# mayataka/robotoc

Measured on AMD Instinct MI355X. Metric: riccati_sweeps_per_sec, higher is better.
Workload: dtype f64; 1 GPU; anymal_trot_N40 (nv=18,nu=12, 47 grids: 2 lifts + 2 impacts, switching constraints ns=6), 4096 DISTINCT OCP instances per GPU (randomised stage data and dx0), backward+forward Riccati sweep; per_gpu_batch=4096, stages=47, parallelism=instances sharded, dp1

## Files before the change

### robotoc_amd/csrc/kernel_set.hpp

```cpp
#pragma once
#include <cstring>

#include "../../include/rtoc.h"
#include "kernel_table.hpp"
#include "condense.hpp"
#include "unconstr_dynamics.hpp"
#include "friction_cone.hpp"
#include "riccati_backward.hpp"
#include "riccati_backward_rs.hpp"
#include "riccati_backward_rv.hpp"
#include "riccati_backward_rw.hpp"
#include "riccati_backward_rw2.hpp"
#include "condense_rv.hpp"
#include "riccati_scan.hpp"
#include "riccati_forward.hpp"
#include "unconstr_riccati.hpp"
#include "parnmpc_backward_correction.hpp"

namespace rtoc {

template <int NV, int NU, int NS, int NW0, int NW1>
inline KernelSet make_set() {
  KernelSet k;
  memset(&k, 0, sizeof(k));
  k.nv = NV;
  k.nu = NU;
  k.ns = NS;
  k.nvariants = 2;
  k.kl = StaticLayout<NV, NU, NS>::make().kkt;
  k.rl = StaticLayout<NV, NU, NS>::make().ric;
  k.bwd[0] = {riccati_backward_kernel<NV, NU, NS, NW0>, 64 * NW0, BwdCfg<NV, NU, NS, NW0>::LDS_BYTES, 1};
  k.bwd[1] = {riccati_backward_kernel<NV, NU, NS, NW1>, 64 * NW1, BwdCfg<NV, NU, NS, NW1>::LDS_BYTES, 1};
  if constexpr (2 * NV + 1 <= 64 && NU + 3 <= 16 && rs_rider_columns_fit<NV>) {
    k.bwd[2] = {riccati_backward_rs_kernel<NV, NU, NS>, 128, BwdCfg<NV, NU, NS, 2>::LDS_BYTES, 1};
    k.nvariants = 3;
    if (4 * BwdCfg<NV, NU, NS, 2>::LDS_BYTES + 64 <= 160 * 1024) {
      k.bwd[3] = {riccati_backward_rs4_kernel<NV, NU, NS>, 512, 4 * BwdCfg<NV, NU, NS, 2>::LDS_BYTES + 64, 4};
      k.nvariants = 4;
      if constexpr (NV % 4 == 2 && NV > NU) k.bwd_sa = {riccati_backward_rs4_kernel<NV, NU, NS, true>, 512, k.bwd[3].lds, 4};
    }
  }
  if constexpr (RvCfg<NV, NU>::OK) {
    k.bwd_rv = {riccati_backward_rv_kernel<NV, NU, NS, false>, 64, rv_lds_bytes<NV, NU, NS>(), 1};
    if constexpr (NV % 16 == 2 && RvCfg<NV, NU>::T == 3 && NV - NU > 0 && NV - NU <= 8 && (NV - NU) % 2 == 0)
    {
      k.bwd_rv_sa = {riccati_backward_rv_kernel<NV, NU, NS, true>, 64, k.bwd_rv.lds, 1};
      k.bwd_rv_sto = {riccati_backward_rv_kernel<NV, NU, NS, true, true>, 64, k.bwd_rv.lds, 1};
    }
  }
  if constexpr (RwCfg<NV, NU>::OK)
    k.bwd_rw = {riccati_backward_rw_kernel<NV, NU, NS>, 64, RwLds<NV, NU, NS>::BYTES, 1};
  else if constexpr (RwCfg<NV, NU>::OK2)
    k.bwd_rw = {riccati_backward_rw2_kernel<NV, NU, NS>, 128, Rw2Lds<NV, NU, NS>::BYTES, 1};
  constexpr int NWF = (2 * NV + NU + 63) / 64;
  if constexpr (NWF == 1)
    k.fwd = {riccati_forward_kernel<NV, NU, NS>, 64, 0, 1};
  else
    k.fwd = {riccati_forward_mw_kernel<NV, NU, NS, NWF>, 64 * NWF, 0, 1};
  k.dl = StaticLayout<NV, NU, NS>::make().dir;
  k.cl = StaticLayout<NV, NU, NS>::make().cdd;
  k.fill = {unconstr_fill_kernel<NV>, 128, 0, 1};
  k.ucond = {unconstr_condense_kernel<NV>, 64, 0, 1};
  k.uexp = {unconstr_expand_kernel<NV>, 64, 0, 1};
  if constexpr (NU == NV && NS == 0 && 2 * NV + 1 <= 64) {
    if constexpr (NV <= 8) k.ubwd = {unconstr_riccati_backward_kernel<NV>, 64, 0, 1};
    else k.ubwd = {unconstr_riccati_backward_lds_kernel<NV>, 64, 0, 1};
    k.ufwd = {unconstr_riccati_forward_kernel<NV>, 64, 0, 1};
  }
  if constexpr (NU == NV && NS == 0 && PbcCfg<NV>::OK) {
    k.pcoarse = {parnmpc_coarse_kernel<NV>, 64, 0, 1};
    k.pcorrect = {parnmpc_correct_kernel<NV>, PBC_CORRECT_NT, 0, 1};
  }
  k.ccond = {cone_condense_kernel<NV, NS>, 64, 0, 1};
  k.cexp = {cone_expand_kernel<NV, NS>, 64, 0, 1};
  k.wcond = {wrench_condense_kernel<NV, NS>, 64, 0, 1};
  k.wexp = {wrench_expand_kernel<NV, NS>, 64, 0, 1};
  constexpr int NF = NS;
  k.cond = {condense_kernel<NV, NU, NF, NS>, CondCfg<NV, NU, NF, NS>::NT, CondCfg<NV, NU, NF, NS>::LDS_BYTES, 1};
  k.cond_split = {condense_kernel<NV, NU, NF, NS, true>, CondCfg<NV, NU, NF, NS>::NT, CondCfg<NV, NU, NF, NS, true>::LDS_BYTES, 1};
  k.mjt = {mjtjinv_kernel<NV, NU, NF, NS>, 64, MjCfg<NV, NF>::LDS_BYTES, 1};
  k.cond_fuses_cones = CondCfg<NV, NU, NF, NS>::FUSE ? 1 : 0;
  k.cond_fused_default = (CondCfg<NV, NU, NF, NS>::FUSE && CondCfg<NV, NU, NF, NS>::ITEMS >= 5) ? 1 : 0;
  if constexpr (CrvCfg<NV, NU, NF, NS>::OK) {
    k.cond_rv = {condense_rv_kernel<NV, NU, NF, NS>, 64, CrvCfg<NV, NU, NF, NS>::LDS_BYTES, 1};
    k.cond_rv_nc = {condense_rv_kernel<NV, NU, NF, NS, false>, 64, CrvCfg<NV, NU, NF, NS>::LDS_BYTES, 1};
    k.cond_rv_cones = CrvCfg<NV, NU, NF, NS>::CONES ? 1 : 0;
  }
  static_assert(!(NV == 18 && NU == 12 && NS == 12) ||
                    (CondCfg<NV, NU, NF, NS, true>::ITEMS >= 5 && CondCfg<NV, NU, NF, NS, true>::MIN_WAVES == 4 && MjCfg<NV, NF>::ITEMS >= 10),
                "LDS carve of the split condensation grew past its granule budget");
  k.expd = {expand_kernel<NV, NU, NF, NS>, 64, ExpCfg<NV, NU, NF>::LDS_BYTES, 1};
  k.scan_elt = {scan_element_kernel<NV, NU, NS>, SCAN_ELT_NT, scan::ElementCfg<NV, NU, NS>::LDS_BYTES, 1};
  k.scan_comb = {scan_combine_kernel<NV>, scan_comb_nt(NV), scan::CombineCfg<NV, scan_comb_nt(NV)>::LDS_BYTES, 1};
  k.scan_elt_stride = scan::EltLayout<NV>::STRIDE;
  k.scan_ps_stride = scan::EltLayout<NV>::PS_STRIDE;
  k.scan_ps_soff = scan::EltLayout<NV>::PS_S;
  k.scan_policy_variant = 1;
  k.fscan_elt = {fwd_scan_element_kernel<NV, NU, NS>, SCAN_FWD_NT, scan::FwdCfg<NV, NU>::LDS_BYTES, 1};
  k.fscan_comb = {fwd_scan_combine_kernel<NV, NU, NS>, SCAN_FWD_NT, scan::FwdCfg<NV, NU>::LDS_BYTES, 1};
  k.fscan_fin = {fwd_scan_finish_kernel<NV, NU, NS>, 64, 0, 1};
  k.sto_prep = {scan_sto_prep_kernel<NV, NU, NS>, SCAN_STO_PREP_NT, scan::StoPrepCfg<NV, NU, NS>::LDS_DOUBLES * (int)sizeof(double), 1};
  k.sto_vec = {scan_sto_vector_kernel<NV, NU, NS>, scan_sto_vec_nt(NV), scan::StoVecCfg<NV, NU, NS>::LDS_BYTES, 1};
  k.sto_scr_stride = scan::StoScratch<NV, NU, NS>::STRIDE;
  static_assert(scan::StoVecCfg<NV, NU, NS>::LDS_BYTES <= 160 * 1024, "the vector pass keeps one grid point's bundle in LDS");
  static_assert(scan::StoVecCfg<NV, NU, NS>::MAX_STAGES == SCAN_STO_MAX_STAGES, "the host's limit (kernel_args.hpp) is the kernel's grid table");
  static_assert(scan::CombineCfg<NV, scan_comb_nt(NV)>::LDS_BYTES <= 160 * 1024, "combination scratch must fit the LDS of a CU");
  return k;
}


// ... 2 lines not shown
```

### robotoc_amd/csrc/kernel_table.hpp

```cpp
#pragma once
#include <cstddef>

#include "kernel_args.hpp"

namespace rtoc {

template <class Args>
struct Kern {
  void (*fn)(Args);
  int threads;
  int lds;
  int inst;
  constexpr explicit operator bool() const { return fn != nullptr; }
};
constexpr size_t kernel_abi_stamp() {
  size_t h = 1469598103934665603ull;
  const size_t parts[] = {sizeof(BwdArgs), sizeof(FwdArgs), sizeof(FillArgs), sizeof(UdArgs), sizeof(ConeArgs), sizeof(CondArgs),
                          sizeof(ExpArgs), sizeof(ScanArgs), sizeof(FwdScanArgs), sizeof(UrArgs), sizeof(StoScanArgs),
                          sizeof(PbcArgs), sizeof(Kern<BwdArgs>)};
  for (size_t v : parts) h = (h ^ v) * 1099511628211ull;
  return h;
}

struct alignas(8) ShapeInfo {
  int nv, nu, ns;
  int nvariants;
  rtoc_record_layout kl, rl, dl, cl;
  int cond_fuses_cones;
  int cond_fused_default;
  int cond_rv_cones;
  int scan_elt_stride, scan_ps_stride, scan_ps_soff;
  int scan_policy_variant;
  int sto_scr_stride;
};
struct KernelSet : ShapeInfo {
  Kern<BwdArgs> bwd[4];
  Kern<BwdArgs> bwd_sa;
  Kern<BwdArgs> bwd_rv;
  Kern<BwdArgs> bwd_rv_sa;
  Kern<BwdArgs> bwd_rv_sto;
  Kern<BwdArgs> bwd_rw;
  Kern<FwdArgs> fwd;
  Kern<FillArgs> fill;
  Kern<UdArgs> ucond, uexp;
  Kern<UrArgs> ubwd, ufwd;
  Kern<ConeArgs> ccond, cexp;
  Kern<ConeArgs> wcond, wexp;
  Kern<CondArgs> cond;
  Kern<CondArgs> cond_split, mjt;
  Kern<CondArgs> cond_rv;
  Kern<CondArgs> cond_rv_nc;
  Kern<ExpArgs> expd;
  Kern<ScanArgs> scan_elt, scan_comb;
  Kern<FwdScanArgs> fscan_elt, fscan_comb, fscan_fin;
  Kern<StoScanArgs> sto_prep, sto_vec;
  Kern<PbcArgs> pcoarse, pcorrect;
};

template <class Set, class F>
constexpr void for_each_kernel(Set& k, F&& f) {
  for (auto& b : k.bwd) f(b);
  f(k.bwd_sa), f(k.bwd_rv), f(k.bwd_rv_sa), f(k.bwd_rv_sto), f(k.bwd_rw);
  f(k.fwd), f(k.fill), f(k.ucond), f(k.uexp), f(k.ubwd), f(k.ufwd);
  f(k.ccond), f(k.cexp), f(k.wcond), f(k.wexp);
  f(k.cond), f(k.cond_split), f(k.mjt), f(k.cond_rv), f(k.cond_rv_nc), f(k.expd);
  f(k.scan_elt), f(k.scan_comb), f(k.fscan_elt), f(k.fscan_comb), f(k.fscan_fin), f(k.sto_prep), f(k.sto_vec);
  f(k.pcoarse), f(k.pcorrect);
}
constexpr size_t kernels_visited() {
  KernelSet k{};
  size_t n = 0;
  for_each_kernel(k, [&n](const auto&) { ++n; });
  return n;
}
static_assert(sizeof(Kern<BwdArgs>) == sizeof(Kern<StoScanArgs>) && sizeof(KernelSet) == sizeof(ShapeInfo) + kernels_visited() * sizeof(Kern<BwdArgs>),
              "for_each_kernel must visit every descriptor of KernelSet (and KernelSet hold nothing else: plain fields go into ShapeInfo)");

}
```

### robotoc_amd/csrc/riccati_forward.hpp

```cpp
#pragma once
#include "device_utils.hpp"
#include "kernel_args.hpp"
#include "../../include/rtoc.h"

namespace rtoc {

#ifndef FWD_PREFETCH
#define FWD_PREFETCH 12
#endif
#ifndef FWD_WAVES_PER_SIMD
#define FWD_WAVES_PER_SIMD 2
#endif

template <int NV, int NU>
struct FwdPairCfg {
  static constexpr int NX = 2 * NV;
  static constexpr int G = 64 / NV;
  static constexpr int TX = (NX + G - 1) / G;
  static constexpr int TXP = (TX + 1) & ~1;
  static constexpr int TK = (NU + G - 1) / G;
  static constexpr int NVP = (NV + 1) & ~1;
  static constexpr int NF = NV * NU, NFP = (NF + 1) & ~1;
  static constexpr int TF = (NFP + 127) / 128;
};

template <int NWF>
__device__ __forceinline__ void fwd_sync() {
  if constexpr (NWF == 1)
    asm volatile("s_waitcnt lgkmcnt(0)" ::: "memory");
  else
    asm volatile("s_waitcnt lgkmcnt(0)\n\ts_barrier" ::: "memory");
}

template <int NV, int NU, int NS>
__global__ __launch_bounds__(64, FWD_WAVES_PER_SIMD) void riccati_forward_kernel(FwdArgs a) {
  using C = FwdPairCfg<NV, NU>;
  constexpr int NX = C::NX, G = C::G, TX = C::TX, TXP = C::TXP, TK = C::TK, NVP = C::NVP, NF = C::NF, TF = C::TF;
  constexpr int PF = FWD_PREFETCH < TX ? FWD_PREFETCH : TX;
  static_assert(NX + NU <= 64, "one lane per row of [Fxx; K] in the reductions");
  __shared__ __attribute__((aligned(16))) double sDx[2][NX + 8];
  __shared__ __attribute__((aligned(16))) double sXp[2][G * TXP];
  __shared__ __attribute__((aligned(16))) double sPa[G + 1][NX];
  __shared__ __attribute__((aligned(16))) double sPp[G + 1][NX];
  __shared__ __attribute__((aligned(16))) double sPk[NX + NU + 1][NVP];
  __shared__ __attribute__((aligned(16))) double sF[TF * 128];
  __shared__ double sDu[NU + 8];
  __shared__ double sDt[NX];
  __shared__ double sRed[8];
  extern __shared__ int sGridTab[];
  const int tid = threadIdx.x;
  const int b = a.first + blockIdx.x;
  if (b >= a.batch) return;
  for (int st = tid; st < a.nstages; st += 64) {
    const rtoc_grid* gp = a.grid + st;
    sGridTab[st] = (gp->type & 15) | ((gp->sto != 0) << 4) | ((gp->sto_next != 0) << 5) |
                   ((gp->switching_constraint != 0) << 6) | (gp->dims << 8);
  }
  for (int e = tid; e < 2 * G * TXP; e += 64) (&sXp[0][0])[e] = 0.0;
  const int N = a.nstages - 1;
  constexpr rtoc_layout SL = StaticLayout<NV, NU, NS>::make();
  constexpr rtoc_record_layout KL = SL.kkt, RL = SL.ric, DL = SL.dir;
  const double* kb = a.kkt + (size_t)b * a.nstages * KL.stride;
  const double* rb = a.ric + (size_t)b * a.nstages * RL.stride;
  double* db = a.dir + (size_t)b * a.nstages * DL.stride;

  const bool lg = tid < G * NV;
  const int p = lg ? tid % NV : tid - G * NV;
  const int c = lg ? tid / NV : 0;
  const int cw = lg ? c : G;
  const bool xrow = tid < NX;
  const int r = xrow ? tid : NX - 1;
  const bool kl = tid >= NX && tid < NX + NU;
  const int u = kl ? tid - NX : 0;
  const int pos = (r % G) * TXP + r / G;
  __syncthreads();
  if (xrow) {
    const double v = a.dx0 ? a.dx0[(size_t)b * NX + tid] : db[DL.off[RTOC_DIR_DX] + tid];
    sDx[0][tid] = v;
    sXp[0][pos] = v;
    if (a.dx0) db[DL.off[RTOC_DIR_DX] + tid] = v;
  }
  __syncthreads();
  double dts = 0.0, dtsn = 0.0;
  {
    const rtoc_grid g0 = a.grid[0];
    if (g0.sto) {
      if (tid == 0) {
        double acc = 0.0;
        for (int k = 0; k < NX; ++k) acc += rb[RL.off[RTOC_RIC_DTSDX] + k] * sDx[0][k];
        sRed[0] = acc + rb[RL.off[RTOC_RIC_SCAL] + RTOC_RIC_SCAL_DTS0];
      }
      __syncthreads();
      dtsn = sRed[0];
      __syncthreads();
    }
  }
  const int lo = c * NX + 2 * p;
  auto moff = [&](int t) { return (NX % G == 0 || t < TX - 1 || G * t + c < NX) ? lo + t * (G * NX) : (NX - 1) * NX + 2 * p; };
  auto live = [&](int t) { return NX % G == 0 || t < TX - 1 || G * t + c < NX; };
  auto koff = [&](int t) { return (NU % G == 0 || t < TK - 1 || G * t + c < NU) ? lo + t * (G * NX) : (NU - 1) * NX + 2 * p; };
  auto klive = [&](int t) { return NU % G == 0 || t < TK - 1 || G * t + c < NU; };
  const int pe = lg ? c - 2 * p : (1 << 20);
  constexpr unsigned P_SILENT = 0x80000000u;
  const auto prsrc = __builtin_amdgcn_make_buffer_rsrc(const_cast<double*>(rb), 0, a.nstages * (int)RL.stride * 8, 0x00020000);
  const int prow = tid < NX + NU ? tid : NX + NU;
  auto vec_ptr = [&](int st) {
    return xrow ? kb + (size_t)st * KL.stride + KL.off[RTOC_KKT_FX] + tid : rb + (size_t)st * RL.stride + RL.off[RTOC_RIC_KV] + u;
  };
  auto s_ptr = [&](int st) { return rb + (size_t)st * RL.stride + RL.off[RTOC_RIC_S] + r; };
  d2 fa[TX];
  double vec, sv;
#pragma unroll
  for (int t = 0; t < PF; ++t) fa[t] = *(const d2*)(kb + KL.off[RTOC_KKT_FXX] + moff(t));
  vec = *vec_ptr(0);
  sv = *s_ptr(0);
  int cur = 0;
  struct GridBits { int type, sto, sto_next, switching_constraint, dims; };
  for (int st = 0; st < N; ++st) {
    const int gb = __builtin_amdgcn_readfirstlane(sGridTab[st]);
    const GridBits g = {gb & 15, (gb >> 4) & 1, (gb >> 5) & 1, (gb >> 6) & 1, gb >> 8};
    const bool impact = g.type == RTOC_GRID_IMPACT, lift = g.type == RTOC_GRID_LIFT;
    const bool sto = g.sto != 0, sto_next = g.sto_next != 0;
    const double* kr = kb + (size_t)st * KL.stride;
    const double* rr = rb + (size_t)st * RL.stride;
    double* dr = db + (size_t)st * DL.stride;
    const double* dx = sDx[cur];
    const double* xp = sXp[cur];

    if (impact || lift) {
      dts = dtsn;
      dtsn = 0.0;
      if (lift && sto_next) {
        if (tid == 0) {
          double acc = 0.0;
          #pragma unroll 4
          for (int k = 0; k < NX; ++k) acc += rr[RL.off[RTOC_RIC_DTSDX] + k] * dx[k];
          acc += rr[RL.off[RTOC_RIC_SCAL] + RTOC_RIC_SCAL_DTS0];
          if (sto) acc += rr[RL.off[RTOC_RIC_SCAL] + RTOC_RIC_SCAL_DTSDTS] * dts;
          sRed[0] = acc;
        }
        fwd_sync<1>();
        dtsn = sRed[0];
        fwd_sync<1>();
      }
    }

    d2 fk[TK], ff[TF], fp[TX];
#pragma unroll
    for (int t = PF; t < TX; ++t) fa[t] = *(const d2*)(kr + KL.off[RTOC_KKT_FXX] + moff(t));
#pragma unroll
    for (int t = 0; t < TK; ++t) fk[t] = *(const d2*)(rr + RL.off[RTOC_RIC_K] + koff(t));
#pragma unroll
    for (int i = 0; i < TF; ++i) {
      const int e = 2 * (64 * i + tid);
      ff[i] = *(const d2*)(kr + KL.off[RTOC_KKT_FVU] + (e < NF ? e : 0));
    }
    double rd1 = 0.0, rd2 = 0.0, rd3 = 0.0, rdt = 0.0, rs0 = 0.0, rss = 0.0;
    if (sto) {
      rd1 = xrow ? kr[KL.off[RTOC_KKT_FFX] + tid] : rr[RL.off[RTOC_RIC_T] + u];
      rd2 = xrow ? rr[RL.off[RTOC_RIC_PSI] + tid] : rr[RL.off[RTOC_RIC_W] + u];
      rd3 = rr[RL.off[RTOC_RIC_PHI] + r];
    }
    if (impact && sto_next) {
      rdt = rr[RL.off[RTOC_RIC_DTSDX] + r];
      rs0 = rr[RL.off[RTOC_RIC_SCAL] + RTOC_RIC_SCAL_DTS0];
      rss = rr[RL.off[RTOC_RIC_SCAL] + RTOC_RIC_SCAL_DTSDTS];
    }
    d2 x[TXP / 2];
#pragma unroll
    for (int i = 0; i < TXP / 2; ++i) x[i] = *(const d2*)(xp + c * TXP + 2 * i);
    const d2 xq = *(const d2*)(dx + 2 * p);
    double a0 = 0.0, a1 = 0.0;
#pragma unroll
    for (int t = 0; t < TX; ++t) {
      const double xt = x[t / 2][t % 2];
      if (live(t)) {
        a0 += fa[t].x * xt;
        a1 += fa[t].y * xt;
      }
    }
    __builtin_amdgcn_sched_barrier(0);
#pragma unroll
    for (int t = 0; t < TX; ++t) {
      const unsigned vo = (pe + G * t <= 1) ? (unsigned)(lo + t * (G * NX)) * 8u : P_SILENT;
      fp[t] = __builtin_bit_cast(d2, __builtin_amdgcn_raw_buffer_load_b128(prsrc, vo, (unsigned)(st * (int)RL.stride + (int)RL.off[RTOC_RIC_P]) * 8u, 0));
    }
    double pk[TK];
#pragma unroll
    for (int t = 0; t < TK; ++t) pk[t] = fk[t].x * xq.x + fk[t].y * xq.y;
#pragma unroll
    for (int i = 0; i < TF; ++i) *(d2*)(sF + 2 * (64 * i + tid)) = ff[i];
    double q0 = 0.0, q1 = 0.0;
#pragma unroll
    for (int t = 0; t < TX; ++t) {
      const double xt = x[t / 2][t % 2];
      const int dd = pe + G * t;
      const double o0 = q0 + fp[t].x * xt, o1 = q1 + fp[t].y * xt;
      q0 = dd <= 0 ? o0 : q0;
      q1 = dd <= 1 ? o1 : q1;
      const double m1 = fp[t].y * xq.y, m01 = m1 + fp[t].x * xq.x;
      sPk[lg && live(t) ? G * t + c : NX + NU][p] = dd < 0 ? m01 : (dd < 1 ? m1 : 0.0);
    }
    double vec_n, sv_n;
    __builtin_amdgcn_sched_barrier(0);
    {
      const double* kn = kb + (size_t)(st + 1) * KL.stride;
#pragma unroll
      for (int t = 0; t < PF; ++t) fa[t] = *(const d2*)(kn + KL.off[RTOC_KKT_FXX] + moff(t));
      vec_n = *vec_ptr(st + 1);
      sv_n = *s_ptr(st + 1);
    }
    {
      d2 va = {a0, a1}, vp = {q0, q1};
      *(d2*)(&sPa[cw][2 * p]) = va;
      *(d2*)(&sPp[cw][2 * p]) = vp;
#pragma unroll
      for (int t = 0; t < TK; ++t) sPk[lg && klive(t) ? NX + G * t + c : NX + NU][p] = pk[t];
    }
    fwd_sync<1>();
    double acc_a = sPa[0][r], acc_p = sPp[0][r];
#pragma unroll
    for (int cc = 1; cc < G; ++cc) {
      acc_a += sPa[cc][r];
      acc_p += sPp[cc][r];
    }
    double kd = 0.0;
#pragma unroll 3
    for (int i = 0; i < NVP / 2; ++i) {
      const d2 w = *(const d2*)(&sPk[prow][2 * i]);
      kd += w.x;
      if (2 * i + 1 < NV) kd += w.y;
    }
    acc_p += xrow ? kd : 0.0;
    if (kl && !impact) {
      double du = kd + vec;
      if (sto) {
        du += rd1 * (dtsn - dts);
        if (sto_next) du -= rd2 * dtsn;
      }
      sDu[u] = du;
      dr[DL.off[RTOC_DIR_DU] + u] = du;
    }
    fwd_sync<1>();
    double* dxn = sDx[cur ^ 1];
    if (xrow) {
      double v = vec + acc_a;
      if (!impact) {
        if (tid >= NV) {
#pragma unroll 4
          for (int cc = 0; cc < NU; ++cc) v += sF[cc * NV + tid - NV] * sDu[cc];
        }
        if (sto) v += rd1 * (dtsn - dts);
      }
      dxn[tid] = v;
      if (impact && sto_next) sDt[tid] = rdt;
      sXp[cur ^ 1][pos] = v;
      (dr + DL.stride)[DL.off[RTOC_DIR_DX] + tid] = v;
    }
    if (impact && sto_next) {
      fwd_sync<1>();
      if (tid == 0) {
        double acc = 0.0;
        #pragma unroll 4
        for (int k = 0; k < NX; ++k) acc += sDt[k] * dxn[k];
        acc += rs0;
        if (sto) acc += rss * dts;
        sRed[0] = acc;
      }
      fwd_sync<1>();
      dtsn = sRed[0];
    }
    if (xrow) {
      double lam = acc_p - sv;
      if (sto) {
        if (impact) {
          lam -= rd3 * dtsn;
        } else {
          lam += rd2 * (dtsn - dts);
          if (sto_next) lam -= rd3 * dtsn;
        }
      }
      dr[DL.off[RTOC_DIR_DLMDGMM] + tid] = lam;
    }
    if (NS > 0 && g.switching_constraint && tid < g.dims) {
      const double* M = rr + RL.off[RTOC_RIC_M] + tid;
      double acc = 0.0;
      #pragma unroll 4
      for (int j = 0; j < NX; ++j) acc += M[j * NS] * dx[j];
      acc += rr[RL.off[RTOC_RIC_MV] + tid];
      if (sto) {
        acc += rr[RL.off[RTOC_RIC_MT] + tid] * (dtsn - dts);
        if (sto_next) acc -= rr[RL.off[RTOC_RIC_MTN] + tid] * dtsn;
      }
      dr[DL.off[RTOC_DIR_DXI] + tid] = acc;
    }
    if (tid == 0) {
      dr[DL.off[RTOC_DIR_DTS] + 0] = dts;
      dr[DL.off[RTOC_DIR_DTS] + 1] = dtsn;
    }
    fwd_sync<1>();
    cur ^= 1;
    vec = vec_n;
    sv = sv_n;
  }
  {
    const double* rr = rb + (size_t)N * RL.stride;
    double* dr = db + (size_t)N * DL.stride;
    const double* xp = sXp[cur];
    d2 fp[TX], x[TXP / 2];
// ... 213 lines not shown
```

### robotoc_amd/csrc/rt_context.hpp

```cpp
#pragma once
#include <hip/hip_runtime.h>

#include <cstdio>
#include <cstdlib>
#include <cstring>
#include <memory>
#include <new>
#include <string>
#include <vector>

#include "../../include/rtoc.h"
#include "../../include/rtoc_robot.h"
#include "device_buffer.hpp"
#include "kernel_table.hpp"
#include "record_view.hpp"
#include "rigid_body_model.hpp"

#define HIP_TRY(expr)                                 \
  do {                                                \
    hipError_t e_ = (expr);                           \
    if (e_ != hipSuccess) {                           \
      rtoc::ctx_set_err(e_, __FILE_NAME__, __LINE__); \
      return RTOC_ERR_HIP;                            \
    }                                                 \
// ... 41 lines not shown
  CtxStreams() = default;
  CtxStreams(const CtxStreams&) = delete;
  CtxStreams& operator=(const CtxStreams&) = delete;
  ~CtxStreams() {
    if (ev0) (void)hipEventDestroy(ev0);
    if (ev1) (void)hipEventDestroy(ev1);
    if (own_stream) (void)hipStreamDestroy(own_stream);
    if (stream2) (void)hipStreamDestroy(stream2);
    if (ev_fork) (void)hipEventDestroy(ev_fork);
    if (ev_join) (void)hipEventDestroy(ev_join);
    for (hipEvent_t e : ev_chunk)
      if (e) (void)hipEventDestroy(e);
  }
};
struct CtxOptions {
  int writeback = 0;
  double max_dts0 = 0.1;
  double contact_inv_damping = 0.0;
  int bwd_variant = 0;
  int sweep_chunks = 1;
  int condense_split = 0;
  int keep_qaf = 0;
  int fxx_mode = 0;
  int bwd_register = 1;
  int cond_register = 1;
  int use_graph = 0;
  int exact_transport = 0;
  int unconstr_dense = 0;
  int exact_cone_jacobian = 0;
  int impact_cones = 1;
  int linearize_fused = 0;
  int lin_dpp = 0;
  double barrier = 0.0, ftb_rule = 0.0;
  int n_mu = 0;
  bool has_cpos = false, has_crot = false;
  int ls_on = 0;
  double ls_rate = 0.0, ls_min_step = 0.0, ls_cost_rate = 0.0, ls_viol_rate = 0.0;
  int ls_method = 0;
  double ls_armijo = 0.0, ls_margin = 0.0, ls_eps = 0.0;
};
struct GraphSlot {
  hipGraphExec_t exec = nullptr;
  unsigned long long epoch = 0, warm_epoch = 0;
  double p0 = 0.0, p1 = 0.0;
  bool warm = false;
  ~GraphSlot() {
    if (exec) (void)hipGraphExecDestroy(exec);
  }
};


struct SweepState {
  int fxx_state = 0;
  BwdPlan bwd_plan;
  DevBuf<int> d_fxx_flag;
  int backward_scan = 0;
  DevBuf<double> d_scan[3];
  DevBuf<double> d_scan_sto;
};

struct ConstraintState {
  DevBuf<double> d_bounds;
  DevBuf<double> d_mu;
  DevBuf<double> d_wcone;
  void clone_from(const ConstraintState& src, CopyChain& dup) {
    dup(d_bounds, src.d_bounds);
    dup(d_mu, src.d_mu);
    dup(d_wcone, src.d_wcone);
  }
  DevBuf<rtoc_box_row> d_rows;
  std::vector<rtoc_box_row> h_rows;
  DevBuf<int> d_pair;
  DevBuf<int> d_entry;
  int nrows = 0;
  int cone_contacts = 0, cone_dim = 0;
  int cone_rows = 0;
};

struct ModelState {
  DevBuf<rbd::DevModel> d_model;
  std::unique_ptr<rbd::DevModel> h_model;
  DevBuf<unsigned> d_active;
  bool active_current = false;
  DevBuf<double> d_cpos;
  DevBuf<double> d_crot;
  DevBuf<double> d_cost;
  DevBuf<double> d_x0;
  DevBuf<double> d_qtab;
  DevBuf<int> d_qtab_active;
  int qtab_on = 0, qtab_n = 0, qtab_inst = 0;
  bool clone_from(const ModelState& src, CopyChain& dup) {
    if (src.h_model) {
      h_model.reset(new (std::nothrow) rbd::DevModel(*src.h_model));
      if (!h_model) return false;
      dup(d_model, src.d_model);
      if (dup.e == hipSuccess) dup.e = set_linearize_lds(h_model->m, h_model->nlevels, h_model->nbranch, h_model->dpp);
    }
    dup(d_active, src.d_active);
    active_current = src.active_current;
    dup(d_cpos, src.d_cpos);
    dup(d_crot, src.d_crot);
    dup(d_cost, src.d_cost);
    dup(d_x0, src.d_x0);
    qtab_on = src.qtab_on, qtab_n = src.qtab_n, qtab_inst = src.qtab_inst;
    dup(d_qtab, src.d_qtab);
    dup(d_qtab_active, src.d_qtab_active);
    return true;
// ... 240 lines not shown
```

### robotoc_amd/csrc/rt_sweep.hip

```cpp
#include "rt_context.hpp"
#include "fxx_structure.hpp"

using namespace rtoc;

static bool grid_has_sto(const rtoc_ctx* c) {
  for (int i = 0; i < c->nstages; ++i)
    if (c->h_grid[i].sto || c->h_grid[i].sto_next) return true;
  return false;
}
static bool scan_applies(const rtoc_ctx* c) {
  if (!c->backward_scan || c->h_grid.empty()) return false;
  if (c->backward_scan == 2 && c->batch > RTOC_SCAN_AUTO_MAX_BATCH) return false;
  if (c->nstages > SCAN_STO_MAX_STAGES && grid_has_sto(c)) return false;
  return true;
}
static bool forward_scan_applies(const rtoc_ctx* c) { return scan_applies(c) && !grid_has_sto(c); }

int rtoc::ensure_scan_buffers(rtoc_ctx* c) {
  const KernelSet* ks = c->ks;
  const size_t per = (size_t)c->batch * c->max_stages;
  for (int i = 0; i < 3; ++i) HIP_TRY(c->d_scan[i].reserve(per * (i < 2 ? ks->scan_elt_stride : ks->scan_ps_stride)));
  if (grid_has_sto(c)) HIP_TRY(c->d_scan_sto.reserve(per * ks->sto_scr_stride));
  return RTOC_OK;
}
// ... 31 lines not shown
  s.batch = end;
  s.first = first;
  s.dist = 0;
  launch(ks->scan_elt, dim3(n, nb), stream, s);
  int cur = 0;
  for (int d = 1; d < n; d *= 2) {
    s.src = c->d_scan[cur].p;
    s.dst = c->d_scan[cur ^ 1].p;
    s.dist = d;
    launch(ks->scan_comb, dim3(n - d, nb, 2), stream, s);
    cur ^= 1;
  }
  BwdArgs a = bwd_args(c, first, end);
  a.prof = nullptr;
  a.scan_ps = c->d_scan[2].p;
  a.scan_ps_stride = ks->scan_ps_stride;
  a.scan_ps_soff = ks->scan_ps_soff;
  const bool sto = grid_has_sto(c);
  StoScanArgs t;
  const bool ride = sto && !c->writeback && ks->sto_prep.lds <= p.kern->lds;
  if (sto) {
    t.kkt = c->buf[RTOC_BUF_KKT].p, t.ric = c->buf[RTOC_BUF_RIC].p, t.grid = c->d_grid.p, t.status = c->d_status.p;
    t.ps = c->d_scan[2].p, t.scr = c->d_scan_sto.p;
    t.nstages = n, t.batch = end, t.first = first, t.max_dts0 = c->max_dts0, t.prof = c->d_prof.p;
    if (!ride) launch(ks->sto_prep, dim3(n - 1, nb), stream, t);
  }
  a.sto_scr = ride ? c->d_scan_sto.p : nullptr;
  launch(*p.kern, dim3(nb, ride ? 2 * n - 1 : n), stream, a);
  if (sto) launch(ks->sto_vec, dim3(nb), stream, t);
  HIP_TRY(hipGetLastError());
  return RTOC_OK;
}

static int check_fxx(rtoc_ctx* c) {
  HIP_TRY(c->d_fxx_flag.reserve(1));
  HIP_TRY(hipMemsetAsync(c->d_fxx_flag.p, 0, sizeof(int), c->stream));
  FxxCheckArgs a;
  a.kkt = c->buf[RTOC_BUF_KKT].p;
  a.grid = c->d_grid.p;
  a.flag = c->d_fxx_flag.p;
  a.nstages = c->nstages;
  a.batch = c->batch;
  a.nv = c->dims.nv;
  a.np = c->dims.np;
  a.fxx_off = c->L.kkt.off[RTOC_KKT_FXX];
  a.stride = c->L.kkt.stride;
  hipLaunchKernelGGL(fxx_structure_kernel, dim3(c->batch * (c->nstages - 1)), dim3(64), 0, c->stream, a);
  HIP_TRY(hipGetLastError());
  int bad = 1;
  HIP_TRY(hipMemcpyAsync(&bad, c->d_fxx_flag.p, sizeof(int), hipMemcpyDeviceToHost, c->stream));
  HIP_TRY(hipStreamSynchronize(c->stream));
  c->fxx_state = bad ? 2 : 1;
  return RTOC_OK;
}

int rtoc::plan_backward(rtoc_ctx* c, BwdPlan* out) {
  const KernelSet* ks = c->ks;
  const bool reg = c->bwd_register && !c->h_grid.empty() && c->nstages >= 2 && c->nstages <= RV_MAX_STAGES && !c->writeback &&
                   c->bwd_variant == default_bwd_variant(ks);
  const bool sto = reg && grid_has_sto(c);
  const bool rw = reg && ks->bwd_rw && !sto && (c->bwd_register >= 2 || c->batch > c->num_cus);
  const bool rewritable = c->fxx_mode == 0 && (!c->buf[RTOC_BUF_KKT].owned || c->kkt_exposed);
  int rc = RTOC_OK;
  auto structured = [&]() {
    if (!((ks->bwd_sa && c->bwd_variant == 3) || rw) || c->fxx_mode == 1) return false;
    if (c->fxx_mode == 2) return true;
    if (c->fxx_state == 0 && rc == RTOC_OK) rc = check_fxx(c);
    return c->fxx_state == 1;
  };
  BwdPlan p = {BWD_TILE, nullptr, 0};
  if (scan_applies(c)) {
    p = {BWD_SCAN, &ks->bwd[ks->scan_policy_variant], 0};
  } else if (reg && ks->bwd_rv && (!sto || (ks->bwd_rv_sto && structured()))) {
    p.path = BWD_RV;
    p.kern = sto ? &ks->bwd_rv_sto : (ks->bwd_rv_sa && structured()) ? &ks->bwd_rv_sa : &ks->bwd_rv;
    p.check_fxx = (p.kern != &ks->bwd_rv && rewritable) ? 1 : 0;
  } else {
    if (rw && rewritable) c->fxx_state = 0;
    const bool s = structured();
    p.path = (rw && s) ? BWD_RW : BWD_TILE;
    p.kern = (rw && s) ? &ks->bwd_rw : s ? &ks->bwd_sa : &ks->bwd[c->bwd_variant];
  }
  if (rc) return rc;
  if (p.path != c->bwd_plan.path || p.kern != c->bwd_plan.kern || p.check_fxx != c->bwd_plan.check_fxx) c->epoch++;
  c->bwd_plan = *out = p;
  return RTOC_OK;
}

static int launch_backward_rv(rtoc_ctx* c, const BwdPlan& p, int first, int end, hipStream_t stream) {
  const int N = c->nstages - 1;
  BwdArgs a = bwd_args(c, first, end);
  a.seg_hi = N - 1;
  a.seg_lo = 0;
  a.check_fxx = p.check_fxx;
#ifdef RTOC_RV_DEBUG_MASK
  if (const char* e = getenv("RTOC_RV_DEBUG")) a.scan_ps_soff = atoi(e);
#endif
  if (N >= 1) launch(*p.kern, dim3(end - first), stream, a);
  HIP_TRY(hipGetLastError());
  return RTOC_OK;
}

static int launch_backward_rw(rtoc_ctx* c, const BwdPlan& p, int first, int end, hipStream_t stream) {
  const KernelSet* ks = c->ks;
  const int N = c->nstages - 1, nb = end - first;
  BwdArgs a = bwd_args(c, first, end);
  auto constrained = [&](int st) { return c->h_grid[st].type != RTOC_GRID_IMPACT && c->h_grid[st].dims > 0; };
  auto one_stage = [&](int st) {
    BwdArgs o = a;
    o.scan_ps = c->buf[RTOC_BUF_RIC].p + c->L.ric.off[RTOC_RIC_P];
    o.scan_ps_stride = c->L.ric.stride;
    o.scan_ps_soff = c->L.ric.off[RTOC_RIC_S] - c->L.ric.off[RTOC_RIC_P];
    o.seg_hi = o.seg_lo = st;
    launch(ks->bwd[ks->scan_policy_variant], dim3(nb, 1), stream, o);
  };
  if (N == 0 || constrained(N - 1)) one_stage(N);
  int hi = N - 1;
  while (hi >= 0) {
    if (constrained(hi)) {
      one_stage(hi);
      --hi;
      continue;
    }
    int lo = hi;
    while (lo > 0 && !constrained(lo - 1)) --lo;
    a.seg_hi = hi;
    a.seg_lo = lo;
    launch(*p.kern, dim3(nb), stream, a);
    hi = lo - 1;
  }
  HIP_TRY(hipGetLastError());
  return RTOC_OK;
}

static int launch_backward_tile(rtoc_ctx* c, const BwdPlan& p, int first, int end, hipStream_t stream) {
  launch(*p.kern, dim3((end - first + p.kern->inst - 1) / p.kern->inst), stream, bwd_args(c, first, end));
  HIP_TRY(hipGetLastError());
  return RTOC_OK;
// ... 1 lines not shown

static int launch_backward_range(rtoc_ctx* c, const BwdPlan& p, int first, int end, hipStream_t stream) {
  switch (p.path) {
    case BWD_SCAN: return launch_backward_scan(c, p, first, end, stream);
    case BWD_RV: return launch_backward_rv(c, p, first, end, stream);
    case BWD_RW: return launch_backward_rw(c, p, first, end, stream);
    default: return launch_backward_tile(c, p, first, end, stream);
  }
}
int rtoc::launch_backward(rtoc_ctx* c, const BwdPlan& p) { return launch_backward_range(c, p, 0, c->batch, c->stream); }

static int launch_forward_scan(rtoc_ctx* c, int first, int end, hipStream_t stream) {
  const KernelSet* ks = c->ks;
  int rc0 = ensure_scan_buffers(c);
  if (rc0) return rc0;
  const int n = c->nstages, nb = end - first, N = n - 1;
  FwdScanArgs s;
  s.kkt = c->buf[RTOC_BUF_KKT].p;
  s.ric = c->buf[RTOC_BUF_RIC].p;
  s.dir = c->buf[RTOC_BUF_DIR].p;
  s.dx0 = c->buf[RTOC_BUF_DX0].p;
  s.grid = c->d_grid.p;
  s.src = c->d_scan[1].p;
  s.dst = c->d_scan[0].p;
  s.nstages = n;
  s.batch = end;
  s.first = first;
  s.dist = 0;
  launch(ks->fscan_elt, dim3(N, nb), stream, s);
  int cur = 0;
  for (int d = 1; d < N; d *= 2) {
    s.src = c->d_scan[cur].p;
    s.dst = c->d_scan[cur ^ 1].p;
    s.dist = d;
    launch(ks->fscan_comb, dim3(N - d, nb), stream, s);
    cur ^= 1;
  }
  launch(ks->fscan_fin, dim3(n, nb), stream, s);
  HIP_TRY(hipGetLastError());
  return RTOC_OK;
}

static int launch_forward_range(rtoc_ctx* c, int first, int end, hipStream_t stream) {
  if (forward_scan_applies(c)) return launch_forward_scan(c, first, end, stream);
  FwdArgs a;
  a.kkt = c->buf[RTOC_BUF_KKT].p;
  a.ric = c->buf[RTOC_BUF_RIC].p;
  a.dir = c->buf[RTOC_BUF_DIR].p;
  a.dx0 = c->buf[RTOC_BUF_DX0].p;
  a.grid = c->d_grid.p;
  a.nstages = c->nstages;
  a.batch = end;
  a.first = first;
  launch(c->ks->fwd, dim3(end - first), stream, a, ((a.nstages + 3) & ~3) * (int)sizeof(int));
  HIP_TRY(hipGetLastError());
  return RTOC_OK;
}
int rtoc::launch_forward(rtoc_ctx* c) { return launch_forward_range(c, 0, c->batch, c->stream); }

int rtoc::launch_sweep(rtoc_ctx* c, const BwdPlan& p) {
  const int nch = (c->sweep_chunks > 0) ? c->sweep_chunks : 1;
  if (nch == 1 || p.path == BWD_SCAN) {
    int rc = launch_backward(c, p);
    return rc ? rc : launch_forward(c);
  }
  const int per = (((c->batch + nch - 1) / nch) + 3) & ~3;
  HIP_TRY(hipEventRecord(c->ev_fork, c->stream));
  HIP_TRY(hipStreamWaitEvent(c->stream2, c->ev_fork, 0));
  for (int i = 0; i * per < c->batch; ++i) {
    const int first = i * per, end = (first + per < c->batch) ? first + per : c->batch;
    int rc = launch_backward_range(c, p, first, end, c->stream);
    if (rc) return rc;
    hipEvent_t e = c->ev_chunk[i % RTOC_MAX_CHUNK_EVENTS];
    HIP_TRY(hipEventRecord(e, c->stream));
    HIP_TRY(hipStreamWaitEvent(c->stream2, e, 0));
    rc = launch_forward_range(c, first, end, c->stream2);
    if (rc) return rc;
  }
  HIP_TRY(hipEventRecord(c->ev_join, c->stream2));
  HIP_TRY(hipStreamWaitEvent(c->stream, c->ev_join, 0));
  return RTOC_OK;
}

int rtoc_riccati_backward(rtoc_ctx* c) {
  CHECK_READY(c);
  BwdPlan p;
  int rc = plan_backward(c, &p);
  return rc ? rc : launch_backward(c, p);
}

int rtoc_riccati_forward(rtoc_ctx* c) {
  CHECK_READY(c);
  return launch_forward(c);
}

int rtoc_graph_replay_count(rtoc_ctx* c, unsigned long long* out) {
  if (!c || !out) return RTOC_ERR_BAD_ARG;
  *out = c->graph_replays;
  return RTOC_OK;
}

int rtoc_riccati_sweep(rtoc_ctx* c) {
  CHECK_READY(c);
  BwdPlan p;
  int rc = plan_backward(c, &p);
  return rc ? rc : run_graphed(c, &c->g_sweep, 0.0, 0.0, [&]() { return launch_sweep(c, p); });
}
// ... 92 lines not shown
```

### robotoc_amd/csrc/rtoc_capi.hip

```cpp
#include <dlfcn.h>

#include "rt_context.hpp"
#include "device_utils.hpp"

using namespace rtoc;

static thread_local char g_errbuf[256] = "";
void rtoc::ctx_set_err(hipError_t e, const char* file, int line) {
  snprintf(g_errbuf, sizeof(g_errbuf), "HIP error %d (%s) at %s:%d", (int)e, hipGetErrorString(e), file, line);
}

int rtoc_version(void) { return 100; }

int rtoc_device_count(void) {
  int n = 0;
  if (hipGetDeviceCount(&n) != hipSuccess) return 0;
  return n;
}

template <int U, bool COPY>
static __global__ __launch_bounds__(256) void stream_probe_kernel(const char* __restrict__ src, char* __restrict__ dst, size_t chunks,
                                                                  double* sink) {
  const size_t nwaves = (size_t)gridDim.x * 4, w = (size_t)blockIdx.x * 4 + (threadIdx.x >> 6);
  const int lane = threadIdx.x & 63;
// ... 140 lines not shown
}

int rtoc_create(const rtoc_dims* dims, int max_stages, int batch, int device, rtoc_ctx** out) {
  if (!dims || !out || max_stages < 2 || batch < 1) return RTOC_ERR_BAD_ARG;
  const KernelSet* ks = find_set(dims);
  if (!ks) return RTOC_ERR_UNSUPPORTED_DIMS;
  if (rtoc_device_count() <= device || device < 0) return RTOC_ERR_NO_DEVICE;
  HIP_TRY(hipSetDevice(device));
  rtoc_ctx* c = new (std::nothrow) rtoc_ctx();
  if (!c) return RTOC_ERR_BAD_ARG;
  c->device = device;
  int rc = create_members(c, dims, ks, max_stages, batch, device);
  if (rc) {
    (void)rtoc_destroy(c);
    return rc;
  }
  *out = c;
  return RTOC_OK;
}

int rtoc_destroy(rtoc_ctx* c) {
  if (!c) return RTOC_ERR_BAD_ARG;
  (void)hipSetDevice(c->device);
  if (c->stream) (void)hipStreamSynchronize(c->stream);
  delete c;
  return RTOC_OK;
}

int rtoc_clone(rtoc_ctx* c, rtoc_ctx** out) {
  if (!c || !out) return RTOC_ERR_BAD_ARG;
  rtoc_ctx* n = nullptr;
  int rc = rtoc_create(&c->dims, c->max_stages, c->batch, c->device, &n);
  if (rc) return rc;
  if (c->parnmpc) rc = rtoc_parnmpc_set_horizon(n, c->nstages);
  else if (c->nstages >= 2 && !c->h_grid.empty()) rc = rtoc_set_grid(n, c->h_grid.data(), c->nstages);
  if (!rc && c->nrows > 0 && !c->h_rows.empty()) rc = rtoc_set_constraint_rows(n, c->h_rows.data(), c->nrows);
  if (!rc && c->cone_contacts > 0)
    rc = c->cone_rows == RTOC_WRENCH_ROWS ? rtoc_set_wrench_cones(n, c->cone_contacts)
                                          : rtoc_set_friction_cones(n, c->cone_contacts, c->cone_dim);
  if (!rc) {
    static_cast<CtxOptions&>(*n) = *c;
    if (c->backward_scan) rc = rtoc_set_option(n, RTOC_OPT_BACKWARD_SCAN, c->backward_scan);
  }
  CopyChain dup{n->stream, hipStreamSynchronize(c->stream)};
  if (!rc && !n->ModelState::clone_from(*c, dup)) rc = RTOC_ERR_HIP;
  if (!rc) {
    n->ConstraintState::clone_from(*c, dup);
    n->LineSearchState::clone_from(*c, dup);
    n->StoState::clone_from(*c, dup);
    n->TaskState::clone_from(*c, dup);
    n->ParnmpcState::clone_from(*c, dup);
    n->InterpState::clone_from(*c, dup);
    n->clone_records(*c, dup);
    if (dup.e == hipSuccess) dup.e = hipStreamSynchronize(n->stream);
  }
  if (rc || dup.e != hipSuccess) {
    if (dup.e != hipSuccess) ctx_set_err(dup.e, __FILE_NAME__, __LINE__);
    (void)rtoc_destroy(n);
    return rc ? rc : RTOC_ERR_HIP;
  }
  *out = n;
  return RTOC_OK;
}

int rtoc_get_layout(const rtoc_ctx* c, rtoc_layout* out) {
  if (!c || !out) return RTOC_ERR_BAD_ARG;
  *out = c->L;
  return RTOC_OK;
}

int rtoc_set_grid(rtoc_ctx* c, const rtoc_grid* grid, int nstages) {
  if (!c || !grid || nstages < 2 || nstages > c->max_stages) return RTOC_ERR_BAD_ARG;
  if (grid[nstages - 1].type != RTOC_GRID_TERMINAL) return RTOC_ERR_BAD_ARG;
  for (int i = 0; i < nstages; ++i) {
    const rtoc_grid& g = grid[i];
    if (g.dims < 0 || g.dims > c->dims.ns_max || g.dimf < 0 || g.dimf > c->dims.nf_max)
      return RTOC_ERR_BAD_ARG;
    if (i < nstages - 1 && g.type == RTOC_GRID_TERMINAL) return RTOC_ERR_BAD_ARG;
    if (g.type == RTOC_GRID_IMPACT && (i == 0 || i >= nstages - 2)) return RTOC_ERR_BAD_ARG;
    if (g.type == RTOC_GRID_LIFT && i == 0) return RTOC_ERR_BAD_ARG;
  }
  HIP_TRY(hipSetDevice(c->device));
  HIP_TRY(hipMemcpyAsync(c->d_grid.p, grid, sizeof(rtoc_grid) * nstages, hipMemcpyHostToDevice, c->stream));
  {
    std::vector<int> list;
    for (int i = 0; i + 1 < nstages; ++i)
      if (grid[i].type != RTOC_GRID_IMPACT) list.push_back(i);
    c->n_stage_contact = (int)list.size();
    for (int i = 0; i + 1 < nstages; ++i)
      if (grid[i].type == RTOC_GRID_IMPACT) list.push_back(i);
    c->n_stage_impact = (int)list.size() - c->n_stage_contact;
    HIP_TRY(hipMemcpyAsync(c->d_stage_list.p, list.data(), sizeof(int) * list.size(), hipMemcpyHostToDevice, c->stream));
    HIP_TRY(hipStreamSynchronize(c->stream));
  }
  HIP_TRY(hipStreamSynchronize(c->stream));
  const bool same = !c->parnmpc && (int)c->h_grid.size() == nstages && c->nstages == nstages &&
                    memcmp(c->h_grid.data(), grid, sizeof(rtoc_grid) * nstages) == 0;
  if (!same) c->active_current = false, c->dt_current = false;
  c->h_grid.assign(grid, grid + nstages);
  c->nstages = nstages;
  c->parnmpc = 0;
  c->fxx_state = 0;
  c->epoch++;
  if (c->sto_on) {
    int nev = 0;
    for (int i = 0; i + 1 < nstages; ++i)
// ... 396 lines not shown
```

Before: 1.593 million sweeps/s.

## Add structured-Fxx forward Riccati kernel exploiting the sparse state-transition block pattern

Adds a forward-sweep kernel variant that uses the known block structure of Fxx when NP = NV - NU is small and even. It loads only the dense bottom rows and a few corner columns through buffer loads, and takes the identity-like middle rows from two scalar coefficients. This replaces the full dense Fxx·dx product. The variant is selected at plan time when the backward plan already uses a structured kernel or the Fxx check confirms the structure. The aim is to cut global loads and FMAs in the forward sweep, at the cost of extra LDS scatter/reduce bookkeeping and reliance on the structure check being correct.

```diff
diff --git a/robotoc_amd/csrc/kernel_set.hpp b/robotoc_amd/csrc/kernel_set.hpp
--- a/robotoc_amd/csrc/kernel_set.hpp
+++ b/robotoc_amd/csrc/kernel_set.hpp
@@ -53,9 +53,11 @@
   else if constexpr (RwCfg<NV, NU>::OK2)
     k.bwd_rw = {riccati_backward_rw2_kernel<NV, NU, NS>, 128, Rw2Lds<NV, NU, NS>::BYTES, 1};
   constexpr int NWF = (2 * NV + NU + 63) / 64;
-  if constexpr (NWF == 1)
+  if constexpr (NWF == 1) {
     k.fwd = {riccati_forward_kernel<NV, NU, NS>, 64, 0, 1};
-  else
+    if constexpr (NV % 16 == 2 && NV - NU > 0 && NV - NU <= 8 && FwdSfCfg<NV, NU>::OK)
+      k.fwd_sf = {riccati_forward_kernel<NV, NU, NS, true>, 64, 0, 1};
+  } else
     k.fwd = {riccati_forward_mw_kernel<NV, NU, NS, NWF>, 64 * NWF, 0, 1};
   k.dl = StaticLayout<NV, NU, NS>::make().dir;
   k.cl = StaticLayout<NV, NU, NS>::make().cdd;
diff --git a/robotoc_amd/csrc/kernel_table.hpp b/robotoc_amd/csrc/kernel_table.hpp
--- a/robotoc_amd/csrc/kernel_table.hpp
+++ b/robotoc_amd/csrc/kernel_table.hpp
@@ -41,6 +41,7 @@
   Kern<BwdArgs> bwd_rv_sto;
   Kern<BwdArgs> bwd_rw;
   Kern<FwdArgs> fwd;
+  Kern<FwdArgs> fwd_sf;
   Kern<FillArgs> fill;
   Kern<UdArgs> ucond, uexp;
   Kern<UrArgs> ubwd, ufwd;
@@ -61,7 +62,7 @@
 constexpr void for_each_kernel(Set& k, F&& f) {
   for (auto& b : k.bwd) f(b);
   f(k.bwd_sa), f(k.bwd_rv), f(k.bwd_rv_sa), f(k.bwd_rv_sto), f(k.bwd_rw);
-  f(k.fwd), f(k.fill), f(k.ucond), f(k.uexp), f(k.ubwd), f(k.ufwd);
+  f(k.fwd), f(k.fwd_sf), f(k.fill), f(k.ucond), f(k.uexp), f(k.ubwd), f(k.ufwd);
   f(k.ccond), f(k.cexp), f(k.wcond), f(k.wexp);
   f(k.cond), f(k.cond_split), f(k.mjt), f(k.cond_rv), f(k.cond_rv_nc), f(k.expd);
   f(k.scan_elt), f(k.scan_comb), f(k.fscan_elt), f(k.fscan_comb), f(k.fscan_fin), f(k.sto_prep), f(k.sto_vec);
diff --git a/robotoc_amd/csrc/riccati_forward.hpp b/robotoc_amd/csrc/riccati_forward.hpp
--- a/robotoc_amd/csrc/riccati_forward.hpp
+++ b/robotoc_amd/csrc/riccati_forward.hpp
@@ -24,6 +24,19 @@
   static constexpr int TF = (NFP + 127) / 128;
 };
 
+template <int NV, int NU>
+struct FwdSfCfg {
+  static constexpr int NX = 2 * NV, NP = NV - NU;
+  static constexpr int HP = NV / 2;
+  static constexpr int GB = 64 / HP;
+  static constexpr int TB = (NX + GB - 1) / GB;
+  static constexpr int TBP = (TB + 1) & ~1;
+  static constexpr int CP = NP >= 2 ? NP / 2 : 1, CC = 2 * NP;
+  static constexpr int NCL = CP * CC;
+  static constexpr int BOT = NP * CC, ZERO = BOT + NV * CC, DROP = ZERO + CC, SPA = DROP + 2 * CC;
+  static constexpr bool OK = NV % 2 == 0 && NP > 0 && NP % 2 == 0 && NCL + 2 <= 64 && CC >= GB;
+};
+
 template <int NWF>
 __device__ __forceinline__ void fwd_sync() {
   if constexpr (NWF == 1)
@@ -32,15 +45,20 @@
     asm volatile("s_waitcnt lgkmcnt(0)\n\ts_barrier" ::: "memory");
 }
 
-template <int NV, int NU, int NS>
+template <int NV, int NU, int NS, bool SF = false>
 __global__ __launch_bounds__(64, FWD_WAVES_PER_SIMD) void riccati_forward_kernel(FwdArgs a) {
   using C = FwdPairCfg<NV, NU>;
+  using S = FwdSfCfg<NV, NU>;
+  static_assert(!SF || S::OK, "the structured form needs an even NV and an even NP = NV - NU > 0 whose corners fit one load");
+  constexpr int NP = S::NP, HP = S::HP, GB = S::GB, TB = S::TB, TBP = S::TBP, NCL = S::NCL;
+  constexpr int TA = SF ? TB + 1 : C::TX;
   constexpr int NX = C::NX, G = C::G, TX = C::TX, TXP = C::TXP, TK = C::TK, NVP = C::NVP, NF = C::NF, TF = C::TF;
-  constexpr int PF = FWD_PREFETCH < TX ? FWD_PREFETCH : TX;
+  constexpr int PF = FWD_PREFETCH < TA ? FWD_PREFETCH : TA;
   static_assert(NX + NU <= 64, "one lane per row of [Fxx; K] in the reductions");
   __shared__ __attribute__((aligned(16))) double sDx[2][NX + 8];
   __shared__ __attribute__((aligned(16))) double sXp[2][G * TXP];
-  __shared__ __attribute__((aligned(16))) double sPa[G + 1][NX];
+  __shared__ __attribute__((aligned(16))) double sXb[SF ? 2 : 1][SF ? GB * TBP : 2];
+  __shared__ __attribute__((aligned(16))) double sPa[SF ? 1 : G + 1][SF ? S::SPA : NX];
   __shared__ __attribute__((aligned(16))) double sPp[G + 1][NX];
   __shared__ __attribute__((aligned(16))) double sPk[NX + NU + 1][NVP];
   __shared__ __attribute__((aligned(16))) double sF[TF * 128];
@@ -57,6 +75,10 @@
                    ((gp->switching_constraint != 0) << 6) | (gp->dims << 8);
   }
   for (int e = tid; e < 2 * G * TXP; e += 64) (&sXp[0][0])[e] = 0.0;
+  if constexpr (SF) {
+    for (int e = tid; e < 2 * GB * TBP; e += 64) (&sXb[0][0])[e] = 0.0;
+    for (int e = tid; e < S::SPA; e += 64) sPa[0][e] = 0.0;
+  }
   const int N = a.nstages - 1;
   constexpr rtoc_layout SL = StaticLayout<NV, NU, NS>::make();
   constexpr rtoc_record_layout KL = SL.kkt, RL = SL.ric, DL = SL.dir;
@@ -73,11 +95,13 @@
   const bool kl = tid >= NX && tid < NX + NU;
   const int u = kl ? tid - NX : 0;
   const int pos = (r % G) * TXP + r / G;
+  const int posb = (r % GB) * TBP + r / GB;
   __syncthreads();
   if (xrow) {
     const double v = a.dx0 ? a.dx0[(size_t)b * NX + tid] : db[DL.off[RTOC_DIR_DX] + tid];
     sDx[0][tid] = v;
     sXp[0][pos] = v;
+    if constexpr (SF) sXb[0][posb] = v;
     if (a.dx0) db[DL.off[RTOC_DIR_DX] + tid] = v;
   }
   __syncthreads();
@@ -103,15 +127,37 @@
   const int pe = lg ? c - 2 * p : (1 << 20);
   constexpr unsigned P_SILENT = 0x80000000u;
   const auto prsrc = __builtin_amdgcn_make_buffer_rsrc(const_cast<double*>(rb), 0, a.nstages * (int)RL.stride * 8, 0x00020000);
+  const bool bl = tid < GB * HP;
+  const int pb = bl ? tid % HP : 0, cb = bl ? tid / HP : 0;
+  const bool cl = tid < NCL;
+  const int qc = cl ? tid % S::CP : 0, jc = cl ? tid / S::CP : 0;
+  const int colc = jc < NP ? jc : NV + jc - NP;
+  const auto krsrc = __builtin_amdgcn_make_buffer_rsrc(const_cast<double*>(kb), 0, a.nstages * (int)KL.stride * 8, 0x00020000);
+  const unsigned boff0 = bl ? (unsigned)(cb * NX + NV + 2 * pb) * 8u : P_SILENT;
+  const unsigned boffl = (NX % GB == 0 || GB * (TB - 1) + cb < NX) ? boff0 : P_SILENT;
+  const unsigned coff = cl ? (unsigned)(colc * NX + 2 * qc) * 8u
+                           : (tid < NCL + 2 ? (unsigned)((tid == NCL ? NP : NV + NP) * NX + NP) * 8u : P_SILENT);
+  auto fxx_load = [&](int st, int t) {
+    const unsigned so = (unsigned)(st * (int)KL.stride + (int)KL.off[RTOC_KKT_FXX]) * 8u;
+    return __builtin_bit_cast(d2, t < TB ? __builtin_amdgcn_raw_buffer_load_b128(krsrc, t < TB - 1 ? boff0 : boffl, so + (unsigned)(t * GB * NX * 8), 0)
+                                         : __builtin_amdgcn_raw_buffer_load_b128(krsrc, coff, so, 0));
+  };
+  const int wb = bl ? S::BOT + (2 * pb) * S::CC + cb : S::DROP;
+  const int wc = cl ? (2 * qc) * S::CC + jc : S::DROP;
+  const bool midrow = tid >= NP && tid < NV;
+  const int ra = tid < NP ? tid * S::CC : (xrow && tid >= NV ? S::BOT + (tid - NV) * S::CC : S::ZERO);
   const int prow = tid < NX + NU ? tid : NX + NU;
   auto vec_ptr = [&](int st) {
     return xrow ? kb + (size_t)st * KL.stride + KL.off[RTOC_KKT_FX] + tid : rb + (size_t)st * RL.stride + RL.off[RTOC_RIC_KV] + u;
   };
   auto s_ptr = [&](int st) { return rb + (size_t)st * RL.stride + RL.off[RTOC_RIC_S] + r; };
-  d2 fa[TX];
+  d2 fa[TA];
   double vec, sv;
 #pragma unroll
-  for (int t = 0; t < PF; ++t) fa[t] = *(const d2*)(kb + KL.off[RTOC_KKT_FXX] + moff(t));
+  for (int t = 0; t < PF; ++t) {
+    if constexpr (SF) fa[t] = fxx_load(0, t);
+    else fa[t] = *(const d2*)(kb + KL.off[RTOC_KKT_FXX] + moff(t));
+  }
   vec = *vec_ptr(0);
   sv = *s_ptr(0);
   int cur = 0;
@@ -147,7 +193,10 @@
 
     d2 fk[TK], ff[TF], fp[TX];
 #pragma unroll
-    for (int t = PF; t < TX; ++t) fa[t] = *(const d2*)(kr + KL.off[RTOC_KKT_FXX] + moff(t));
+    for (int t = PF; t < TA; ++t) {
+      if constexpr (SF) fa[t] = fxx_load(st, t);
+      else fa[t] = *(const d2*)(kr + KL.off[RTOC_KKT_FXX] + moff(t));
+    }
 #pragma unroll
     for (int t = 0; t < TK; ++t) fk[t] = *(const d2*)(rr + RL.off[RTOC_RIC_K] + koff(t));
 #pragma unroll
@@ -171,12 +220,32 @@
     for (int i = 0; i < TXP / 2; ++i) x[i] = *(const d2*)(xp + c * TXP + 2 * i);
     const d2 xq = *(const d2*)(dx + 2 * p);
     double a0 = 0.0, a1 = 0.0;
-#pragma unroll
-    for (int t = 0; t < TX; ++t) {
-      const double xt = x[t / 2][t % 2];
-      if (live(t)) {
+    double mid = 0.0;
+    if constexpr (SF) {
+      d2 xb[TBP / 2];
+#pragma unroll
+      for (int i = 0; i < TBP / 2; ++i) xb[i] = *(const d2*)(sXb[cur] + cb * TBP + 2 * i);
+      const double xc = dx[colc];
+      const double xm0 = dx[midrow ? tid : 0], xm1 = dx[midrow ? NV + tid : 0];
+#pragma unroll
+      for (int t = 0; t < TB; ++t) {
+        const double xt = xb[t / 2][t % 2];
         a0 += fa[t].x * xt;
         a1 += fa[t].y * xt;
+      }
+      mid = readlane_d(fa[TB].x, NCL) * xm0 + readlane_d(fa[TB].x, NCL + 1) * xm1;
+      sPa[0][wb] = a0;
+      sPa[0][wb + S::CC] = a1;
+      sPa[0][wc] = fa[TB].x * xc;
+      sPa[0][wc + S::CC] = fa[TB].y * xc;
+    } else {
+#pragma unroll
+      for (int t = 0; t < TX; ++t) {
+        const double xt = x[t / 2][t % 2];
+        if (live(t)) {
+          a0 += fa[t].x * xt;
+          a1 += fa[t].y * xt;
+        }
       }
     }
     __builtin_amdgcn_sched_barrier(0);
@@ -206,24 +275,38 @@
     {
       const double* kn = kb + (size_t)(st + 1) * KL.stride;
 #pragma unroll
-      for (int t = 0; t < PF; ++t) fa[t] = *(const d2*)(kn + KL.off[RTOC_KKT_FXX] + moff(t));
+      for (int t = 0; t < PF; ++t) {
+        if constexpr (SF) fa[t] = fxx_load(st + 1, t);
+        else fa[t] = *(const d2*)(kn + KL.off[RTOC_KKT_FXX] + moff(t));
+      }
       vec_n = *vec_ptr(st + 1);
       sv_n = *s_ptr(st + 1);
     }
     {
       d2 va = {a0, a1}, vp = {q0, q1};
-      *(d2*)(&sPa[cw][2 * p]) = va;
+      if constexpr (!SF) *(d2*)(&sPa[cw][2 * p]) = va;
       *(d2*)(&sPp[cw][2 * p]) = vp;
 #pragma unroll
       for (int t = 0; t < TK; ++t) sPk[lg && klive(t) ? NX + G * t + c : NX + NU][p] = pk[t];
     }
     fwd_sync<1>();
-    double acc_a = sPa[0][r], acc_p = sPp[0][r];
-#pragma unroll
-    for (int cc = 1; cc < G; ++cc) {
-      acc_a += sPa[cc][r];
-      acc_p += sPp[cc][r];
-    }
+    double acc_a, acc_p = sPp[0][r];
+    if constexpr (SF) {
+      acc_a = 0.0;
+#pragma unroll
+      for (int i = 0; i < S::CC / 2; ++i) {
+        const d2 w = *(const d2*)(&sPa[0][ra + 2 * i]);
+        acc_a += w.x;
+        acc_a += w.y;
+      }
+      acc_a = midrow ? mid : acc_a;
+    } else {
+      acc_a = sPa[0][r];
+#pragma unroll
+      for (int cc = 1; cc < G; ++cc) acc_a += sPa[cc][r];
+    }
+#pragma unroll
+    for (int cc = 1; cc < G; ++cc) acc_p += sPp[cc][r];
     double kd = 0.0;
 #pragma unroll 3
     for (int i = 0; i < NVP / 2; ++i) {
@@ -255,6 +338,7 @@
       dxn[tid] = v;
       if (impact && sto_next) sDt[tid] = rdt;
       sXp[cur ^ 1][pos] = v;
+      if constexpr (SF) sXb[cur ^ 1][posb] = v;
       (dr + DL.stride)[DL.off[RTOC_DIR_DX] + tid] = v;
     }
     if (impact && sto_next) {
diff --git a/robotoc_amd/csrc/rt_context.hpp b/robotoc_amd/csrc/rt_context.hpp
--- a/robotoc_amd/csrc/rt_context.hpp
+++ b/robotoc_amd/csrc/rt_context.hpp
@@ -117,7 +117,13 @@
 
 struct SweepState {
   int fxx_state = 0;
+  bool bwd_structured = false;
+  void clone_from(const SweepState& src) {
+    fxx_state = src.fxx_state;
+    bwd_structured = src.bwd_structured;
+  }
   BwdPlan bwd_plan;
+  int fwd_sf = 0;
   DevBuf<int> d_fxx_flag;
   int backward_scan = 0;
   DevBuf<double> d_scan[3];
diff --git a/robotoc_amd/csrc/rt_sweep.hip b/robotoc_amd/csrc/rt_sweep.hip
--- a/robotoc_amd/csrc/rt_sweep.hip
+++ b/robotoc_amd/csrc/rt_sweep.hip
@@ -107,6 +107,13 @@
   HIP_TRY(hipStreamSynchronize(c->stream));
   c->fxx_state = bad ? 2 : 1;
   return RTOC_OK;
+}
+
+static bool forward_structured(const rtoc_ctx* c) {
+  const KernelSet* ks = c->ks;
+  if (!ks->fwd_sf || c->fxx_mode == 1 || c->dims.np != c->dims.nv - c->dims.nu) return false;
+  if (c->fxx_mode == 2 || c->fxx_state == 1) return true;
+  return c->fxx_state == 0 && c->bwd_structured;
 }
 
 int rtoc::plan_backward(rtoc_ctx* c, BwdPlan* out) {
@@ -137,8 +144,12 @@
     p.kern = (rw && s) ? &ks->bwd_rw : s ? &ks->bwd_sa : &ks->bwd[c->bwd_variant];
   }
   if (rc) return rc;
-  if (p.path != c->bwd_plan.path || p.kern != c->bwd_plan.kern || p.check_fxx != c->bwd_plan.check_fxx) c->epoch++;
+  const bool changed = p.path != c->bwd_plan.path || p.kern != c->bwd_plan.kern || p.check_fxx != c->bwd_plan.check_fxx;
   c->bwd_plan = *out = p;
+  c->bwd_structured = p.kern == &ks->bwd_sa || p.kern == &ks->bwd_rv_sa || p.kern == &ks->bwd_rv_sto || (p.path == BWD_RW && p.kern == &ks->bwd_rw);
+  const int sf = forward_structured(c) ? 1 : 0;
+  if (changed || sf != c->fwd_sf) c->epoch++;
+  c->fwd_sf = sf;
   return RTOC_OK;
 }
 
@@ -246,7 +257,8 @@
   a.nstages = c->nstages;
   a.batch = end;
   a.first = first;
-  launch(c->ks->fwd, dim3(end - first), stream, a, ((a.nstages + 3) & ~3) * (int)sizeof(int));
+  const Kern<FwdArgs>& k = forward_structured(c) ? c->ks->fwd_sf : c->ks->fwd;
+  launch(k, dim3(end - first), stream, a, ((a.nstages + 3) & ~3) * (int)sizeof(int));
   HIP_TRY(hipGetLastError());
   return RTOC_OK;
 }
diff --git a/robotoc_amd/csrc/rtoc_capi.hip b/robotoc_amd/csrc/rtoc_capi.hip
--- a/robotoc_amd/csrc/rtoc_capi.hip
+++ b/robotoc_amd/csrc/rtoc_capi.hip
@@ -216,6 +216,7 @@
     n->ParnmpcState::clone_from(*c, dup);
     n->InterpState::clone_from(*c, dup);
     n->clone_records(*c, dup);
+    n->SweepState::clone_from(*c);
     if (dup.e == hipSuccess) dup.e = hipStreamSynchronize(n->stream);
   }
   if (rc || dup.e != hipSuccess) {
```

New measurement: 1.596 million sweeps/s (median of 2 runs). About the same (+0.2%).
